# ceres-solver/ceres-solver

Hardware: NVIDIA H100
Metric: lm_iterations_per_sec (higher is better)
Workload: dtype f64

## Files before the change

ceres_solver_b200/csrc/explicit_schur.cuh:

```cuda
#pragma once
#include "common.cuh"

namespace b200 {

constexpr int kXsThreads = 256;
constexpr int kXsWarps = kXsThreads / 32;
constexpr int kXsMinCtas = 2;
constexpr int kXsStep = 3;
constexpr int kXsAsmThreads = 256;
constexpr int kXsLongPairs = 96;
constexpr int kXsStepCountShift = 27;
constexpr int kXsStepFirst = 1 << 29;
constexpr int kXsStepLast = 1 << 30;

struct XsView {
  int C;
  int num_blocks;
  const int* blk_row;
  const int* blk_col;
  const int* pair_ptr;
  const int2* pairs;
  const int2* cols;
  const int* col_ptr;
  const int2* steps;
// ... 65 lines not shown
                                                                   double* __restrict__ upper45) {
  __shared__ double s_part[kLong ? kXsAsmThreads / 32 : 1][81];
  const int lane = threadIdx.x & 31, warp = threadIdx.x >> 5;
  const bool owner = lane < 27;
  const int u = owner ? lane / 3 : 0, w0 = owner ? 3 * (lane - 3 * (lane / 3)) : 0;
  const int item0 = kLong ? static_cast<int>(blockIdx.x) : static_cast<int>(blockIdx.x) * (kXsAsmThreads / 32) + warp;
  const int items = kLong ? static_cast<int>(gridDim.x) : static_cast<int>(gridDim.x) * (kXsAsmThreads / 32);
  for (int it = item0; it < num; it += items) {
    const int b = __ldg(blocks + it);
    const int p0 = __ldg(v.pair_ptr + b), p1 = __ldg(v.pair_ptr + b + 1);
    double acc[3] = {0.0, 0.0, 0.0};
    if (kLong) {
      constexpr int W = kXsAsmThreads / 32;
      const int n = p1 - p0;
      xs_pairs(v, p, ete_inv, p0 + static_cast<int>(static_cast<long long>(n) * warp / W),
               p0 + static_cast<int>(static_cast<long long>(n) * (warp + 1) / W), lane, acc[0], acc[1], acc[2]);
      __syncthreads();
      if (owner)
#pragma unroll
        for (int m = 0; m < 3; ++m) s_part[warp][9 * u + w0 + m] = acc[m];
      __syncthreads();
      if (warp != 0) continue;
      if (owner)
#pragma unroll
        for (int m = 0; m < 3; ++m) {
          double t = 0.0;
#pragma unroll
          for (int k = 0; k < W; ++k) t += s_part[k][9 * u + w0 + m];
          acc[m] = t;
        }
    } else {
      xs_pairs(v, p, ete_inv, p0, p1, lane, acc[0], acc[1], acc[2]);
    }
    if (owner) {
      double* sb = v.S + 81 * static_cast<size_t>(b) + 9 * u + w0;
      sb[0] = acc[0];
      sb[1] = acc[1];
      sb[2] = acc[2];
      const int i = __ldg(v.blk_row + b);
      if (upper45 != nullptr && __ldg(v.blk_col + b) == i) {
        double* o = upper45 + 45 * static_cast<size_t>(i) + u * 9 - u * (u - 1) / 2 - u;
        if (u <= w0) o[w0] = acc[0];
        if (u <= w0 + 1) o[w0 + 1] = acc[1];
        if (u <= w0 + 2) o[w0 + 2] = acc[2];
      }
    }
  }
}

struct XsStepData {
  int2 d;
  int2 c;
  double s[9];
};
template <bool kShared>
__device__ __forceinline__ int2 xs_step_desc(const XsView& v, int k, int k1) {
  return k < k1 ? (kShared ? v.steps[k] : __ldg(v.steps + k)) : make_int2(0, 0);
}
__device__ __forceinline__ bool xs_lane_in(int2 d, int e) { return e < ((d.y >> kXsStepCountShift) & 3); }
template <bool kShared>
__device__ __forceinline__ int2 xs_step_col(const XsView& v, int2 d, int e) {
  return xs_lane_in(d, e) ? (kShared ? v.cols[d.x + e] : __ldg(v.cols + d.x + e)) : make_int2(0, -1);
}
__device__ __forceinline__ void xs_step_s(const XsView& v, int2 d, int e, int w, double* s) {
  const bool in = xs_lane_in(d, e);
  const int b = in ? d.x + e : 0;
  const double* sb = v.S + 81 * static_cast<size_t>(b) + w;
#pragma unroll
  for (int u = 0; u < 9; ++u) s[u] = in ? __ldg(sb + 9 * u) : 0.0;
}

struct XsWalk {
  XsStepData nx;
  int2 d2, c2;
};
template <bool kShared = false, class LoadS>
__device__ __forceinline__ void xs_walk_begin(const XsView& v, int k0, int k1, int e, int w, LoadS load_s, XsWalk& wk) {
  wk.nx.d = xs_step_desc<kShared>(v, k0, k1);
  wk.nx.c = xs_step_col<kShared>(v, wk.nx.d, e);
  load_s(wk.nx.d, e, w, wk.nx.s);
  wk.d2 = xs_step_desc<kShared>(v, k0 + 1, k1);
  wk.c2 = xs_step_col<kShared>(v, wk.d2, e);
}
template <bool kShared = false, class LoadS, class LoadX, class RowOut>
__device__ __forceinline__ double xs_walk(const XsView& v, int k0, int k1, int lane, int e, int w, LoadS load_s, LoadX load_x,
                                          RowOut row_out, XsWalk& wk) {
  XsStepData& nx = wk.nx;
  int2 d2 = wk.d2, c2 = wk.c2;
  double nx_x = xs_lane_in(nx.d, e) ? load_x(nx.c.x, w) : 0.0;
  double acc[9], xi[9];
#pragma unroll
  for (int u = 0; u < 9; ++u) acc[u] = xi[u] = 0.0;
  double pq = 0.0;
  for (int k = k0; k < k1; ++k) {
    const int2 d = nx.d, c = nx.c;
    double s[9];
#pragma unroll
    for (int u = 0; u < 9; ++u) s[u] = nx.s[u];
    const double xj = nx_x;
    nx.d = d2;
    nx.c = c2;
    load_s(nx.d, e, w, nx.s);
    nx_x = xs_lane_in(nx.d, e) ? load_x(nx.c.x, w) : 0.0;
    d2 = xs_step_desc<kShared>(v, k + 2, k1);
    c2 = xs_step_col<kShared>(v, d2, e);
    if (d.y & kXsStepFirst)
#pragma unroll
      for (int u = 0; u < 9; ++u) xi[u] = __shfl_sync(0xffffffffu, xj, u);
    double t = 0.0;
#pragma unroll
    for (int u = 0; u < 9; ++u) {
      acc[u] += s[u] * xj;
      t += s[u] * xi[u];
    }
    if (c.y >= 0) {
      v.T[9 * static_cast<size_t>(c.y) + w] = t;
      pq += xj * t;
    }
    if (d.y & kXsStepLast) {
      double mine = 0.0, xo = 0.0;
#pragma unroll
      for (int u = 0; u < 9; ++u) {
        double a = acc[u];
#pragma unroll
        for (int o = 16; o > 0; o >>= 1) a += __shfl_xor_sync(0xffffffffu, a, o);
        if (lane == u) {
          mine = a;
          xo = xi[u];
        }
        acc[u] = 0.0;
      }
      if (lane < 9) {
        pq += xo * mine;
        row_out(d.y & ((1 << kXsStepCountShift) - 1), lane, mine, xo);
      }
    }
  }
  return pq;
}

__global__ void __launch_bounds__(kXsThreads, kXsMinCtas) xs_mul_kernel(XsView v, const double* __restrict__ x, double* y,
                                                                        const double* __restrict__ Df, int accumulate,
                                                                        const int* __restrict__ done_flag, double* pq_part) {
  __shared__ double s_pq[kXsWarps];
  const int warp = threadIdx.x >> 5, lane = threadIdx.x & 31;
  const int e = lane / 9, w = lane - 9 * (lane / 9);
  const int gw = blockIdx.x * kXsWarps + warp;
  const int k0 = __ldg(v.warp_step + gw), k1 = __ldg(v.warp_step + gw + 1);
  auto load_s = [&](int2 d, int e, int w, double* s) { xs_step_s(v, d, e, w, s); };
  XsWalk wk;
  xs_walk_begin(v, k0, k1, e, w, load_s, wk);
  asm volatile("griddepcontrol.wait;" ::: "memory");
  if (done_flag != nullptr && __ldcg(done_flag) != 0) return;
  double pq = xs_walk(
      v, k0, k1, lane, e, w, load_s, [&](int j, int w) { return __ldcg(x + 9 * static_cast<size_t>(j) + w); },
      [&](int i, int u, double a, double xo) {
        const size_t o = 9 * static_cast<size_t>(i) + u;
        double out = a;
        if (Df != nullptr) out += Df[o] * Df[o] * xo;
        if (accumulate) out += __ldcg(y + o);
        y[o] = out;
      },
      wk);
  if (pq_part == nullptr) return;
#pragma unroll
  for (int o = 16; o > 0; o >>= 1) pq += __shfl_xor_sync(0xffffffffu, pq, o);
  if (lane == 0) s_pq[warp] = pq;
  __syncthreads();
  if (threadIdx.x == 0) {
    double tot = 0.0;
#pragma unroll
    for (int ww = 0; ww < kXsWarps; ++ww) tot += s_pq[ww];
    pq_part[blockIdx.x] = tot;
  }
}

template <bool kStaged>
__device__ __forceinline__ double xs_col_sum(const double* src, int base, int c0, int c1, int w, double q) {
  for (int c = c0; c < c1; c += 8) {
    double t[8];
#pragma unroll
    for (int m = 0; m < 8; ++m) {
      const double* s = src + 9 * static_cast<size_t>(c + m - base) + w;
      t[m] = c + m < c1 ? (kStaged ? *s : __ldcg(s)) : 0.0;
    }
#pragma unroll
    for (int m = 0; m < 8; ++m)
      if (c + m < c1) q += t[m];
  }
  return q;
}
__device__ __forceinline__ double xs_col_sum(const int* __restrict__ col_ptr, const double* T, int k, double q) {
  const int j = k / 9, w = k - 9 * (k / 9);
  return xs_col_sum<false>(T, 0, __ldg(col_ptr + j), __ldg(col_ptr + j + 1), w, q);
}

__global__ void __launch_bounds__(256) xs_gather_kernel(XsView v, double* y) {
  const int k = blockIdx.x * blockDim.x + threadIdx.x;
  if (k < 9 * v.C) y[k] = xs_col_sum(v.col_ptr, v.T, k, y[k]);
}

}
```

ceres_solver_b200/csrc/plan.cuh:

```cuda
#pragma once
#include <algorithm>
#include <cmath>
#include <cstdio>
#include <cstdlib>
#include <cstring>
#include <numeric>
#include <vector>

#include "explicit_schur.cuh"
#include "kernels_v4b.cuh"
#include "xs_pcg.cuh"

namespace b200 {

constexpr double kL2ResidentShare = 0.5;
constexpr double kXsByteRatio = 2.0;
constexpr double kXsMaxBytes = 128.0 * (1 << 20);

enum KernelId {
  K_EVAL_JAC = 0,
  K_EVAL_COST,
  K_SQNORM,
  K_SCALE,
  K_JMUL,
// ... 64 lines not shown
    if (const char* e = dev_env("B200_BIG_COST")) k.big_cost = std::max(0.0, atof(e));
    if (const char* e = dev_env("B200_DIRECT_LIMIT")) k.direct_limit = atol(e);
    if (const char* e = dev_env("B200_V3_WARPS")) k.v3_warps = atoi(e);
    if (const char* e = dev_env("B200_V3_REPLICAS")) k.v3_replicas = atoi(e);
    if (const char* e = dev_env("B200_V4_WARPS")) k.v4_warps = std::max(4, std::min(k.v4_warps, atoi(e)));
    if (const char* e = dev_env("B200_V4_STAGES")) k.v4_stages = std::max(1, std::min(3, atoi(e)));
    if (const char* e = dev_env("B200_V4_REPLICAS")) k.v4_replicas = std::max(1, atoi(e));
    if (const char* e = dev_env("B200_L2_RESIDENT_MB")) {
      k.l2_mb_set = true;
      k.l2_mb = atof(e);
    }
    if (const char* e = dev_env("B200_L2_RESIDENT_POLICY")) k.l2_last = strcmp(e, "last") == 0;
    if (const char* e = dev_env("B200_EXPLICIT_S")) k.explicit_s = atoi(e) != 0 ? 1 : 0;
    k.no_pdl = dev_env("B200_NO_PDL") != nullptr;
    k.no_fused_pq = dev_env("B200_NO_FUSED_PQ") != nullptr;
    k.no_peer_exchange = dev_env("B200_NO_PEER_EXCHANGE") != nullptr;
    if (const char* e = dev_env("B200_XS_RESIDENT")) k.xs_resident = atoi(e) != 0 ? 1 : 0;
    return k;
  }
};

struct DevLimits {
  int sm_count;
  size_t smem_optin;
  int l2_bytes;
  int xs_ctas_per_sm;
  int xs_pcg_ctas_per_sm;
};

enum class MulFamily { Tile, V3, V4, V4Owned };
enum class DiagPass { CamMajor, WarpTile, Tile };

inline bool is_v4(MulFamily m) { return m == MulFamily::V4 || m == MulFamily::V4Owned; }

struct XsPattern {
  long long off_blocks = 0;
  std::vector<int> blk_row, blk_col, pair_ptr, row_ptr, col_ptr;
  std::vector<int2> pairs, cols;
};

struct KernelPlan {
  int order_choice = 0;
  long order_metrics[4] = {0, 0, 0, 0};
  std::vector<int> pt_perm;
  std::vector<int> row_perm;
  std::vector<int> cam_idx, pt_idx, pt_ptr;
  std::vector<double> obs;
  std::vector<TileDesc> tiles;
  std::vector<TileDesc> chunk_tiles;
  std::vector<int> huge_pts;
  std::vector<WarpTile> wtiles;
  std::vector<TileDesc> big_tiles;
  int num_plain_big = 0;
  std::vector<uint32_t> row_meta;
  std::vector<int> cam_rows;
  std::vector<CamItem> cam_items;
  bool has_dups = false;
  int num_ctas = 0;
  std::vector<int2> cta_part, cta_cam, cta_big;
  std::vector<int> cta_cams;
  int max_cam_span = 1;
  MulFamily mul = MulFamily::Tile;
  DiagPass diag = DiagPass::Tile;
  bool big_folded = false;
  V2View v2{}, v2_mul{}, v2_eval{}, v2_diag{};
  size_t v2_smem = 0, mul_smem = 0, eval_smem = 0, diag_smem = 0;
  int diag_replicas = 0;
  std::vector<uint32_t> tile_meta;
  double l2_budget = 0.0, l2_stream_bytes = 0.0, l2_resident_bytes = 0.0;
  bool xs = false;
  XsPattern xp;
  std::vector<int> xs_order;
  std::vector<int2> xs_steps;
  std::vector<int> xs_warp_step;
  int num_xs_long = 0, xs_grid = 0, xs_resident = 0, xs_max_steps = 0;
  bool xs_pcg = false;
  std::vector<int2> xs_pcg_cta;
  std::vector<int> xs_pcg_warp_step;
  std::vector<int> xs_pcg_fptr;
  std::vector<int> xs_pcg_fcol;
  std::vector<int2> xs_pcg_cols;
  int xs_pcg_max_blocks = 0, xs_pcg_max_cams = 0, xs_pcg_max_steps = 0, xs_pcg_max_foreign = 0;
  int xs_pcg_max_cta_steps = 0;
  int xs_pcg_max_slots = 0;
  int xs_pcg_stage_slots = 0;
  size_t xs_pcg_smem = 0;
  const char* xs_pcg_why = "";
  double bytes_per_op[K_COUNT] = {};
};

inline void xs_pattern(int C, int N, const int* cam_idx, const int* pt_idx, const int* pt_ptr, XsPattern* xp) {
  std::vector<int> cptr(static_cast<size_t>(C) + 1, 0), crow(static_cast<size_t>(N));
  for (int r = 0; r < N; ++r) cptr[cam_idx[r] + 1]++;
  for (int c = 0; c < C; ++c) cptr[c + 1] += cptr[c];
  {
    std::vector<int> fill(cptr.begin(), cptr.end() - 1);
    for (int r = 0; r < N; ++r) crow[fill[cam_idx[r]]++] = r;
  }
  std::vector<int> stamp(static_cast<size_t>(C), -1), slot(static_cast<size_t>(C), 0), js, start;
  std::vector<int>& row_start = xp->row_ptr;
  row_start.assign(static_cast<size_t>(C) + 1, 0);
  std::vector<int3> tup;
  for (int i = 0; i < C; ++i) {
    js.clear();
    tup.clear();
    stamp[i] = i;
    js.push_back(i);
    for (int k = cptr[i]; k < cptr[i + 1]; ++k) {
      const int r = crow[k], p = pt_idx[r];
      for (int s = pt_ptr[p]; s < pt_ptr[p + 1]; ++s) {
        const int j = cam_idx[s];
        if (j < i) continue;
        if (stamp[j] != i) {
          stamp[j] = i;
          js.push_back(j);
        }
        tup.push_back(make_int3(j, r, s));
      }
    }
    std::sort(js.begin(), js.end());
    xp->off_blocks += static_cast<long long>(js.size()) - 1;
    row_start[i] = static_cast<int>(xp->blk_row.size());
    start.assign(js.size() + 1, 0);
    for (size_t t = 0; t < js.size(); ++t) {
      slot[js[t]] = static_cast<int>(t);
      xp->blk_row.push_back(i);
      xp->blk_col.push_back(js[t]);
    }
    for (const int3& t : tup) start[slot[t.x] + 1]++;
    for (size_t t = 0; t < js.size(); ++t) start[t + 1] += start[t];
    const size_t base = xp->pairs.size();
    for (size_t t = 0; t < js.size(); ++t) xp->pair_ptr.push_back(static_cast<int>(base + start[t]));
    xp->pairs.resize(base + tup.size());
    for (const int3& t : tup) xp->pairs[base + start[slot[t.x]]++] = make_int2(t.y, t.z);
  }
  const int nb = static_cast<int>(xp->blk_row.size());
  row_start[C] = nb;
  xp->pair_ptr.push_back(static_cast<int>(xp->pairs.size()));
  xp->col_ptr.assign(static_cast<size_t>(C) + 1, 0);
  for (int b = 0; b < nb; ++b)
    if (xp->blk_col[b] != xp->blk_row[b]) xp->col_ptr[xp->blk_col[b] + 1]++;
  for (int c = 0; c < C; ++c) xp->col_ptr[c + 1] += xp->col_ptr[c];
  std::vector<int> fill(xp->col_ptr.begin(), xp->col_ptr.end() - 1);
  xp->cols.resize(static_cast<size_t>(nb));
  for (int b = 0; b < nb; ++b)
    xp->cols[b] = make_int2(xp->blk_col[b], xp->blk_col[b] != xp->blk_row[b] ? fill[xp->blk_col[b]]++ : -1);
}

inline int xs_assembly_order(const XsPattern& xp, std::vector<int>* order) {
  const int nb = static_cast<int>(xp.blk_row.size());
  order->clear();
  order->reserve(static_cast<size_t>(nb));
  for (int b = 0; b < nb; ++b)
    if (xp.pair_ptr[b + 1] - xp.pair_ptr[b] > kXsLongPairs) order->push_back(b);
  const int num_long = static_cast<int>(order->size());
  for (int b = 0; b < nb; ++b)
    if (xp.pair_ptr[b + 1] - xp.pair_ptr[b] <= kXsLongPairs) order->push_back(b);
  return num_long;
}

const char* const kOrderNames[4] = {"caller's order kept", "by camera arc", "by mean camera", "by smallest camera"};
inline int choose_point_order(int C, int P, int N, const int32_t* cam_of_row, const int* caller_ptr, int chunks, std::vector<int>* perm,
                       long metrics[4]) {
  std::vector<int> ident(static_cast<size_t>(P));
  std::iota(ident.begin(), ident.end(), 0);
  auto metric = [&](const std::vector<int>& ord) -> long {
// ... 440 lines not shown
    if (knobs.explicit_s >= 0) pl.xs = knobs.explicit_s != 0 && npairs < 2.0e9;
    xs_asm_bytes = 196.0 * N + 48.0 * P + 8.0 * npairs + 12.0 * nb + 648.0 * nb + 360.0 * C;
  }
  if (pl.xs) {
    const XsPattern& xp = pl.xp;
    const int nb = static_cast<int>(xp.blk_row.size());
    pl.xs_resident = std::max(1, lim.xs_ctas_per_sm) * lim.sm_count;
    pl.xs_grid = std::max(1, std::min(pl.xs_resident, (C + kXsWarps - 1) / kXsWarps));
    const int nw = pl.xs_grid * kXsWarps;
    auto row_steps = [&](int i) { return (xp.row_ptr[i + 1] - xp.row_ptr[i] + kXsStep - 1) / kXsStep; };
    double total = 0.0;
    for (int i = 0; i < C; ++i) total += row_steps(i) + 1;
    pl.xs_warp_step.assign(static_cast<size_t>(nw) + 1, 0);
    double cum = 0.0;
    int w = 0;
    for (int i = 0; i < C; ++i) {
      const int owner = std::min(nw - 1, static_cast<int>(cum * nw / total));
      while (w < owner) pl.xs_warp_step[++w] = static_cast<int>(pl.xs_steps.size());
      const int r0 = xp.row_ptr[i], r1 = xp.row_ptr[i + 1];
      for (int b = r0; b < r1; b += kXsStep) {
        const int n = std::min(kXsStep, r1 - b);
        pl.xs_steps.push_back(make_int2(b, i | (n << kXsStepCountShift) | (b == r0 ? kXsStepFirst : 0) |
                                               (b + kXsStep >= r1 ? kXsStepLast : 0)));
      }
      cum += row_steps(i) + 1;
    }
    while (w < nw) pl.xs_warp_step[++w] = static_cast<int>(pl.xs_steps.size());
    for (int k = 0; k < nw; ++k) pl.xs_max_steps = std::max(pl.xs_max_steps, pl.xs_warp_step[k + 1] - pl.xs_warp_step[k]);
    {
      const int G = lim.sm_count;
      std::vector<int> first_step(static_cast<size_t>(C) + 1, 0);
      for (int i = 0; i < C; ++i) first_step[i + 1] = first_step[i] + row_steps(i);
      auto row_blocks = [&](int i) { return xp.row_ptr[i + 1] - xp.row_ptr[i]; };
      auto ctas_at = [&](int K) {
        int g = 1, cur = 0;
        for (int i = 0; i < C; ++i) {
          if (cur + row_blocks(i) > K) {
            ++g;
            cur = 0;
          }
          cur += row_blocks(i);
        }
        return g;
      };
      int lo = (nb + G - 1) / G, hi = nb;
      for (int i = 0; i < C; ++i) lo = std::max(lo, row_blocks(i));
      while (lo < hi) {
        const int mid = lo + (hi - lo) / 2;
        if (ctas_at(mid) <= G) hi = mid;
        else lo = mid + 1;
      }
      pl.xs_pcg_cta.assign(static_cast<size_t>(G) + 1, make_int2(C, nb));
      pl.xs_pcg_cta[0] = make_int2(0, 0);
      for (int i = 0, g = 0, cur = 0; i < C; ++i) {
        if (cur + row_blocks(i) > lo) {
          pl.xs_pcg_cta[++g] = make_int2(i, xp.row_ptr[i]);
          cur = 0;
        }
        cur += row_blocks(i);
      }
      pl.xs_pcg_warp_step.assign(static_cast<size_t>(G) * kXpWarps + 1, first_step[C]);
      pl.xs_pcg_fptr.assign(static_cast<size_t>(G) + 1, 0);
      pl.xs_pcg_cols.resize(static_cast<size_t>(nb));
      for (int b = 0; b < G; ++b) {
        const int i0 = pl.xs_pcg_cta[b].x, i1 = pl.xs_pcg_cta[b + 1].x;
        const int b0 = pl.xs_pcg_cta[b].y, b1 = pl.xs_pcg_cta[b + 1].y;
        pl.xs_pcg_max_blocks = std::max(pl.xs_pcg_max_blocks, b1 - b0);
        pl.xs_pcg_max_cams = std::max(pl.xs_pcg_max_cams, i1 - i0);
        pl.xs_pcg_max_cta_steps = std::max(pl.xs_pcg_max_cta_steps, first_step[i1] - first_step[i0]);
        pl.xs_pcg_max_slots = std::max(pl.xs_pcg_max_slots, xp.col_ptr[i1] - xp.col_ptr[i0]);
        std::vector<int> fc;
        for (int k = b0; k < b1; ++k)
          if (xp.blk_col[k] >= i1) fc.push_back(xp.blk_col[k]);
        std::sort(fc.begin(), fc.end());
        fc.erase(std::unique(fc.begin(), fc.end()), fc.end());
        for (int k = b0; k < b1; ++k) {
          const int j = xp.blk_col[k];
          const int l = j < i1 ? j - i0 : (i1 - i0) + static_cast<int>(std::lower_bound(fc.begin(), fc.end(), j) - fc.begin());
          pl.xs_pcg_cols[k] = make_int2(l, xp.cols[k].y);
        }
        pl.xs_pcg_fcol.insert(pl.xs_pcg_fcol.end(), fc.begin(), fc.end());
        pl.xs_pcg_fptr[b + 1] = static_cast<int>(pl.xs_pcg_fcol.size());
        pl.xs_pcg_max_foreign = std::max(pl.xs_pcg_max_foreign, static_cast<int>(fc.size()));
        double tot = 0.0, cum = 0.0;
        for (int i = i0; i < i1; ++i) tot += row_steps(i) + 1;
        int* ws = pl.xs_pcg_warp_step.data() + static_cast<size_t>(b) * kXpWarps;
        int wv = 0;
        ws[0] = first_step[i0];
        for (int i = i0; i < i1; ++i) {
          const int owner = std::min(kXpWarps - 1, static_cast<int>(cum * kXpWarps / tot));
          while (wv < owner) ws[++wv] = first_step[i];
          cum += row_steps(i) + 1;
        }
        while (wv < kXpWarps - 1) ws[++wv] = first_step[i1];
      }
      for (int k = 0; k < G * kXpWarps; ++k)
        pl.xs_pcg_max_steps = std::max(pl.xs_pcg_max_steps, pl.xs_pcg_warp_step[k + 1] - pl.xs_pcg_warp_step[k]);
      const size_t base = xs_pcg_smem_bytes(pl.xs_pcg_max_blocks, pl.xs_pcg_max_cams, pl.xs_pcg_max_foreign, pl.xs_pcg_max_cta_steps, 0);
      const size_t room = lim.smem_optin > base + 1024 ? lim.smem_optin - base - 1024 : 0;
      pl.xs_pcg_stage_slots = static_cast<int>(std::min<size_t>(pl.xs_pcg_max_slots, room / (9 * sizeof(double))));
      pl.xs_pcg_smem = xs_pcg_smem_bytes(pl.xs_pcg_max_blocks, pl.xs_pcg_max_cams, pl.xs_pcg_max_foreign, pl.xs_pcg_max_cta_steps,
                                         pl.xs_pcg_stage_slots);
      if (pl.xs_pcg_smem + 1024 > lim.smem_optin) pl.xs_pcg_why = "largest CTA's shared memory exceeds the limit";
      else if (lim.xs_pcg_ctas_per_sm < 1) pl.xs_pcg_why = "no CTA of the kernel fits an SM";
      else if (knobs.xs_resident == 0) pl.xs_pcg_why = "B200_XS_RESIDENT=0";
      else pl.xs_pcg = true;
    }
    pl.num_xs_long = xs_assembly_order(xp, &pl.xs_order);
  }

  const double Nn = N, Pp = P, Cc = C;
  double* bpo = pl.bytes_per_op;
  bpo[K_JTJ] = 196 * Nn + 4 * Pp + 24.0 * (3 * Pp + 9 * Cc);
  bpo[K_SCHUR_MUL] = 196 * Nn + 52 * Pp + 216 * Cc;
  bpo[K_SCHUR_INIT] = 196 * Nn + 16 * Nn + 4 * Pp + 24 * Pp + 48 * Pp + 72 * Cc;
  bpo[K_DIAG_BLOCKS] = 196 * Nn + 52 * Pp + 360 * Cc;
  bpo[K_BACKSUB] = 196 * Nn + 16 * Nn + 52 * Pp + 24 * Pp + 72 * Cc;
  bpo[K_EVAL_JAC] = 192 * Nn + 16 * Nn + 16 * Nn + 4 * Nn + 4 * Pp + 2 * 8.0 * (3 * Pp + 9 * Cc);
  bpo[K_EVAL_COST] = 16 * Nn + 4 * Nn + 4 * Pp + 8.0 * (3 * Pp + 9 * Cc);
  bpo[K_SQNORM] = 196 * Nn + 4 * Pp + 8.0 * (3 * Pp + 9 * Cc);
  bpo[K_SCALE] = 2 * 192 * Nn + 8 * Nn + 8.0 * (3 * Pp + 9 * Cc);
  bpo[K_JMUL] = 196 * Nn + 32 * Nn + 4 * Pp + 8.0 * (3 * Pp + 9 * Cc);
  bpo[K_JTMUL] = 196 * Nn + 16 * Nn + 4 * Pp + 16.0 * (3 * Pp + 9 * Cc);
  bpo[K_PMV_RIGHT_E] = 48 * Nn + 4 * Nn + 32 * Nn + 24 * Pp;
  bpo[K_PMV_RIGHT_F] = 144 * Nn + 4 * Nn + 32 * Nn + 72 * Cc;
  bpo[K_PMV_LEFT_E] = 48 * Nn + 16 * Nn + 4 * Pp + 48 * Pp;
  bpo[K_PMV_LEFT_F] = 144 * Nn + 16 * Nn + 4 * Nn + 144 * Cc;
  bpo[K_MODEL_COST] = 196 * Nn + 16 * Nn + 4 * Pp + 8.0 * (3 * Pp + 9 * Cc);
  bpo[K_DOGLEG_GRAM] = 196 * Nn + 4 * Pp + 16.0 * (3 * Pp + 9 * Cc);
  bpo[K_DOGLEG_DIAG] = 48.0 * (3 * Pp + 9 * Cc);
  bpo[K_DOGLEG_GN] = 32.0 * (3 * Pp + 9 * Cc);
  bpo[K_DOGLEG_STEP] = 56.0 * (3 * Pp + 9 * Cc);
  if (pl.xs) {
    bpo[K_SCHUR_MUL] = xs_mul_bytes;
    bpo[K_DIAG_BLOCKS] = xs_asm_bytes;
    const double nb = static_cast<double>(pl.xp.blk_row.size()), off = static_cast<double>(pl.xp.off_blocks);
    if (pl.xs_pcg) bpo[K_SCHUR_PCG] = 656.0 * nb + 144.0 * off + 648.0 * Cc + 8 * 72.0 * Cc;
  }
}

inline void print_plan(const KernelPlan& pl, int C, int P, int N, int world, const DevLimits& lim, const DevKnobs& knobs) {
  if (getenv("B200_VERBOSE") == nullptr) return;
  if (!knobs.keep_order)
    fprintf(stderr, "[b200ba] point order: distinct cameras per 1/%d of the rows, summed: caller %ld, by camera arc %ld, by mean camera %ld, by smallest camera %ld -> %s\n",
            lim.sm_count, pl.order_metrics[0], pl.order_metrics[1], pl.order_metrics[2], pl.order_metrics[3], kOrderNames[pl.order_choice]);
  const V2View &v = pl.v2, &m = pl.v2_mul;
  if (is_v4(pl.mul)) {
    const uint32_t s = m.l2_stream;
    fprintf(stderr, "[b200ba] S*x L2 plan (L2 %d MiB, budget %.1f MiB): resident %.1f MiB, streamed %.1f MiB, stride %.2f tiles (%s)\n",
            lim.l2_bytes >> 20, pl.l2_budget / (1 << 20), pl.l2_resident_bytes / (1 << 20), (pl.l2_stream_bytes - pl.l2_resident_bytes) / (1 << 20),
            s < 65536 ? 65536.0 / (65536 - s) : 0.0, m.l2_last ? "evict_last" : "evict_normal");
  }
  const char* const mul_names[] = {"tile", "v3", "v4", "v4-owned"};
  const char* const diag_names[] = {"cam_major", "v2", "tile"};
  fprintf(stderr,
          "[b200ba] C=%d P=%d N=%d wtiles=%zu big(+slices)=%zu huge=%d span=%d direct=%d v2(w=%d,s=%d,r=%d) mul(%s w=%d,s=%d,r=%d,smem=%zu) folded=%d v2b=%d cam_major=%d diag=%s\n",
          C, P, N, pl.wtiles.size(), pl.big_tiles.size(), static_cast<int>(pl.huge_pts.size()), pl.max_cam_span, v.direct, v.warps, v.stages,
          v.replicas, mul_names[static_cast<int>(pl.mul)], m.warps, m.stages, m.replicas, pl.mul_smem, pl.big_folded ? 1 : 0,
          is_v4(pl.mul) ? 1 : 0, pl.diag == DiagPass::CamMajor ? 1 : 0, diag_names[static_cast<int>(pl.diag)]);
  if (world == 1) {
    fprintf(stderr, "[b200ba] S plan: %s, %lld pairs, %.1f MB\n", pl.xs ? "explicit" : "implicit", pl.xp.off_blocks,
            648.0 * static_cast<double>(pl.xp.blk_row.size()) / 1e6);
    if (pl.xs)
      fprintf(stderr, "[b200ba] S product: grid %d of %d resident CTAs (%d per SM), %d warps, at most %d steps per warp\n",
              pl.xs_grid, pl.xs_resident, lim.xs_ctas_per_sm, pl.xs_grid * kXsWarps, pl.xs_max_steps);
    if (pl.xs) {
      const double share = 648.0 * pl.xs_pcg_max_blocks / 1024.0, limit = static_cast<double>(lim.smem_optin) / 1024.0;
      const double cta = static_cast<double>(pl.xs_pcg_smem) / 1024.0;
      if (pl.xs_pcg)
        fprintf(stderr, "[b200ba] S PCG: resident, %d CTAs, largest S share %.2f KiB of %.2f KiB (%.2f KiB with M^-1, vectors and staging), %d warps, at most %d steps per warp, at most %d foreign columns, at most %d column slots per CTA (%d staged)\n",
                lim.sm_count, share, limit, cta, lim.sm_count * kXpWarps, pl.xs_pcg_max_steps, pl.xs_pcg_max_foreign, pl.xs_pcg_max_slots,
                pl.xs_pcg_stage_slots);
      else
        fprintf(stderr, "[b200ba] S PCG: two-kernel (%s: largest S share %.2f KiB, %.2f KiB with M^-1, vectors and staging, of %.2f KiB)\n",
                pl.xs_pcg_why, share, cta, limit);
    }
  } else
    fprintf(stderr, "[b200ba] S plan: implicit, sharded\n");
}

}
```

ceres_solver_b200/csrc/xs_pcg.cuh:

```cuda
#pragma once
#include "cg_kernel.cuh"

namespace b200 {

constexpr int kXpThreads = 512;
constexpr int kXpWarps = kXpThreads / 32;
inline size_t xs_pcg_smem_bytes(int max_blocks, int max_cams, int max_foreign, int max_steps, int slots) {
  return sizeof(double) * (81 * static_cast<size_t>(max_blocks) + (81 + 7 * 9) * static_cast<size_t>(max_cams) +
                           9 * static_cast<size_t>(max_cams + max_foreign) + 9 * static_cast<size_t>(slots)) +
         sizeof(int2) * (static_cast<size_t>(max_steps) + static_cast<size_t>(max_blocks)) +
         sizeof(int) * (static_cast<size_t>(max_cams) + 1 + static_cast<size_t>(max_foreign));
}

struct XsPcgArgs {
  XsView v;
  CgParams prm;
  int reset;
  const int2* cta;
  const int* warp_step;
  const int* fptr;
  const int* fcol;
  int max_blocks, max_cams;
  int max_foreign;
  int max_steps;
  int stage_slots;
  const double* minv;
  const double* rhs;
  const double* Df;
  double *x, *z;
  double* p[2];
  double* red;
  CgState* st;
#ifdef B200_DEV_KNOBS
  long long* stamps;
#endif
};

constexpr int kXpPhases = 6;
#ifdef B200_DEV_KNOBS
#define XP_STAMP(k)                                                   \
  if (a.stamps != nullptr && blockIdx.x == 0 && threadIdx.x == 0) {   \
    const long long t_now = clock64();                                \
    a.stamps[k] += t_now - t_mark;                                    \
    t_mark = t_now;                                                   \
  }
#else
#define XP_STAMP(k)
#endif

__global__ void __launch_bounds__(kXpThreads, 1) xs_pcg_kernel(XsPcgArgs a) {
  cg::grid_group grid = cg::this_grid();
#ifdef B200_DEV_KNOBS
  long long t_mark = clock64();
#endif
  extern __shared__ double smem[];
  __shared__ double scratch[kXpWarps][3];
  __shared__ double s_tot[4];
  __shared__ int s_nfe;
  const int tid = threadIdx.x, warp = tid >> 5, lane = tid & 31;
  const int e = lane / 9, w = lane - 9 * (lane / 9);
  const int2 lo = a.cta[blockIdx.x], hi = a.cta[blockIdx.x + 1];
  const int r0 = lo.x, ncam = hi.x - lo.x, nent = 9 * ncam, b0 = lo.y, nblk = hi.y - lo.y;
  double* s_S = smem;
  double* s_minv = s_S + 81 * static_cast<size_t>(a.max_blocks);
  double* s_x = s_minv + 81 * static_cast<size_t>(a.max_cams);
  double* s_r = s_x + 9 * a.max_cams;
  double* s_p = s_r + 9 * a.max_cams;
  double* s_b = s_p + 9 * a.max_cams;
  double* s_d = s_b + 9 * a.max_cams;
  double* s_a = s_d + 9 * a.max_cams;
  double* s_z = s_a + 9 * a.max_cams;
  double* s_v = s_z + 9 * a.max_cams;
  double* s_T = s_v + 9 * (a.max_cams + a.max_foreign);
  int2* s_steps = reinterpret_cast<int2*>(s_T + 9 * a.stage_slots);
  int2* s_cols = s_steps + a.max_steps;
  int* s_cp = reinterpret_cast<int*>(s_cols + a.max_blocks);
  int* s_fc = s_cp + a.max_cams + 1;
  const XsView& v = a.v;
  const int kc = __ldg(a.warp_step + blockIdx.x * kXpWarps);
  XsView vs = v;
  vs.steps = s_steps - kc;
  vs.cols = s_cols - b0;
  const size_t o0 = 9 * static_cast<size_t>(r0);
  const bool writer = blockIdx.x == 0 && tid == 0;
  const int k0 = __ldg(a.warp_step + blockIdx.x * kXpWarps + warp), k1 = __ldg(a.warp_step + blockIdx.x * kXpWarps + warp + 1);

  {
    const double* src = v.S + 81 * static_cast<size_t>(b0);
    const int n = 81 * nblk;
    int i = tid;
    for (; i + 3 * kXpThreads < n; i += 4 * kXpThreads) {
      double t[4];
#pragma unroll
      for (int k = 0; k < 4; ++k) t[k] = __ldcg(src + i + k * kXpThreads);
#pragma unroll
      for (int k = 0; k < 4; ++k) s_S[i + k * kXpThreads] = t[k];
    }
    for (; i < n; i += kXpThreads) s_S[i] = __ldcg(src + i);
    for (int k = tid; k < 81 * ncam; k += kXpThreads) s_minv[k] = __ldcg(a.minv + 81 * static_cast<size_t>(r0) + k);
    for (int k = tid; k <= ncam; k += kXpThreads) s_cp[k] = __ldg(v.col_ptr + r0 + k);
    const int nsteps = __ldg(a.warp_step + (blockIdx.x + 1) * kXpWarps) - kc;
    for (int k = tid; k < nsteps; k += kXpThreads) s_steps[k] = __ldg(v.steps + kc + k);
    for (int k = tid; k < nblk; k += kXpThreads) s_cols[k] = __ldg(v.cols + b0 + k);
    const int f0 = __ldg(a.fptr + blockIdx.x), nf = __ldg(a.fptr + blockIdx.x + 1) - f0;
    for (int k = tid; k < nf; k += kXpThreads) s_fc[k] = __ldg(a.fcol + f0 + k);
    if (tid == 0) s_nfe = 9 * nf;
  }
  for (int k = tid; k < nent; k += kXpThreads) {
    s_b[k] = a.rhs[o0 + k];
    s_d[k] = a.Df != nullptr ? a.Df[o0 + k] : 0.0;
    s_p[k] = 0.0;
  }
  auto load_s = [&](int2 d, int e, int w, double* s) {
    const bool in = xs_lane_in(d, e);
    const double* sb = s_S + 81 * (in ? d.x + e - b0 : 0) + w;
#pragma unroll
    for (int u = 0; u < 9; ++u) s[u] = in ? sb[9 * u] : 0.0;
  };
  auto keep_row = [&](int i, int u, double av, double) { s_a[9 * (i - r0) + u] = av; };
  auto staged = [&]() { return s_cp[ncam] - s_cp[0] <= a.stage_slots; };
  auto stage_T = [&]() {
    if (!staged()) return;
    const int c0 = s_cp[0];
    const double* src = v.T + 9 * static_cast<size_t>(c0);
    const int n = 9 * (s_cp[ncam] - c0);
    int i = tid;
    for (; i + 7 * kXpThreads < n; i += 8 * kXpThreads) {
      double t[8];
#pragma unroll
      for (int k = 0; k < 8; ++k) t[k] = __ldcg(src + i + k * kXpThreads);
#pragma unroll
      for (int k = 0; k < 8; ++k) s_T[i + k * kXpThreads] = t[k];
    }
    for (; i < n; i += kXpThreads) s_T[i] = __ldcg(src + i);
  };
  auto col_sum = [&](bool from_s, int k, double init) {
    const int cl = k / 9;
    return from_s ? xs_col_sum<true>(s_T, s_cp[0], s_cp[cl], s_cp[cl + 1], k - 9 * cl, init)
                  : xs_col_sum(v.col_ptr, v.T, static_cast<int>(o0) + k, init);
  };
  auto precondition = [&]() {
    __syncthreads();
    double accQ = 0.0, accR = 0.0, accRho = 0.0;
    for (int k = tid; k < nent; k += kXpThreads) {
      const int cl = k / 9, row = k - 9 * cl;
      const double* m = s_minv + 81 * cl + 9 * row;
      const double* rc = s_r + 9 * cl;
      double zj = 0.0;
#pragma unroll
      for (int t = 0; t < 9; ++t) zj += m[t] * rc[t];
      s_z[k] = zj;
      a.z[o0 + k] = zj;
      const double xj = s_x[k], rj = s_r[k];
      accQ += xj * (s_b[k] + rj);
      accR += rj * rj;
      accRho += rj * zj;
    }
    cg_block_sum3<kXpWarps>(accQ, accR, accRho, scratch);
    if (tid == 0) {
      a.red[blockIdx.x * 4 + 1] = accQ;
      a.red[blockIdx.x * 4 + 2] = accR;
      a.red[blockIdx.x * 4 + 3] = accRho;
    }
  };

  for (int k = tid; k < nent; k += kXpThreads) {
    s_x[k] = 0.0;
    s_r[k] = s_b[k];
    a.x[o0 + k] = 0.0;
  }
  precondition();
  grid.sync();
  double tot[3];
  cg_totals(a.red, gridDim.x, 1, 3, tot, s_tot);
  XP_STAMP(0);
  double rho = 1.0, Q0 = 0.0, tol_r = 0.0, beta = 0.0;
  int it = 0;
  if (!cg_phase_c(a.prm, true, 0, rho, Q0, tol_r, tot[0], tot[1], tot[2], a.st, writer, &beta, &Q0, &tol_r)) return;
  rho = tot[2];

  for (;;) {
    double pq = 0.0;
    const double* p_prev = a.p[it & 1];
    for (int k = tid; k < nent + s_nfe; k += kXpThreads) {
      if (k < nent) {
        const double pn = cg_next_p(it, s_z[k], beta, s_p[k]);
        s_p[k] = pn;
        s_v[k] = pn;
        a.p[(it + 1) & 1][o0 + k] = pn;
        pq += s_d[k] * s_d[k] * pn * pn;
      } else {
        const int fl = (k - nent) / 9;
        const size_t o = 9 * static_cast<size_t>(s_fc[fl]) + (k - nent - 9 * fl);
        s_v[k] = cg_next_p(it, __ldcg(a.z + o), beta, __ldcg(p_prev + o));
      }
    }
    ++it;
    __syncthreads();
    {
      XsWalk wk;
      xs_walk_begin<true>(vs, k0, k1, e, w, load_s, wk);
      pq += xs_walk<true>(vs, k0, k1, lane, e, w, load_s, [&](int l, int w) { return s_v[9 * l + w]; }, keep_row, wk);
    }
    {
      double d1 = 0.0, d2 = 0.0;
      cg_block_sum3<kXpWarps>(pq, d1, d2, scratch);
      if (tid == 0) a.red[blockIdx.x * 4] = pq;
    }
    XP_STAMP(1);
    grid.sync();
    XP_STAMP(2);
    double pq_tot, alpha = 0.0;
    const bool reset = it % a.reset == 0;
    if (!reset) stage_T();
    cg_totals(a.red, gridDim.x, 0, 1, &pq_tot, s_tot);
    if (!cg_alpha(pq_tot, rho, it, a.st, writer, &alpha)) return;
    const bool from_s = staged();
    for (int k = tid; k < nent; k += kXpThreads) {
      const double pj = s_p[k];
      double xj = s_x[k];
      xj += alpha * pj;
      s_x[k] = xj;
      a.x[o0 + k] = xj;
      if (reset) {
        s_v[k] = xj;
      } else {
        const double dj = s_d[k];
        const double q = col_sum(from_s, k, __dadd_rn(s_a[k], __dmul_rn(__dmul_rn(dj, dj), pj)));
        double rj = s_r[k];
        rj -= alpha * q;
        s_r[k] = rj;
      }
    }
    if (reset) {
      grid.sync();
      for (int k = tid; k < s_nfe; k += kXpThreads) {
        const int fl = k / 9;
        s_v[nent + k] = __ldcg(a.x + 9 * static_cast<size_t>(s_fc[fl]) + (k - 9 * fl));
      }
      __syncthreads();
      {
        XsWalk wk;
        xs_walk_begin<true>(vs, k0, k1, e, w, load_s, wk);
        xs_walk<true>(vs, k0, k1, lane, e, w, load_s, [&](int l, int w) { return s_v[9 * l + w]; }, keep_row, wk);
      }
      grid.sync();
      stage_T();
      __syncthreads();
      for (int k = tid; k < nent; k += kXpThreads) {
        const double dj = s_d[k];
        const double q = col_sum(from_s, k, __dadd_rn(s_a[k], __dmul_rn(__dmul_rn(dj, dj), s_x[k])));
        s_r[k] = s_b[k] - q;
      }
    }
    precondition();
    XP_STAMP(3);
    grid.sync();
    XP_STAMP(4);
    cg_totals(a.red, gridDim.x, 1, 3, tot, s_tot);
    if (!cg_phase_c(a.prm, false, it, rho, Q0, tol_r, tot[0], tot[1], tot[2], a.st, writer, &beta, &Q0, &tol_r)) return;
    rho = tot[2];
    XP_STAMP(5);
  }
}

}
```

Baseline: 142.7.

## Split Schur rows across warps with segment joins, transpose smem S, prefetch foreign p

The persistent PCG kernel now gives each warp a balanced share of steps, found by binary search on a per-step cost. A row may be split across warps, so partial row sums go to a per-warp segment buffer and are joined after the walk. It also stores the S blocks transposed in shared memory so the per-lane loads are contiguous, and prefetches the foreign z/p values into registers right after the grid sync. This aims to cut warp load imbalance and shared-memory bank conflicts, at the cost of extra join logic, shared memory and synchronisation.

```diff
diff --git a/ceres_solver_b200/csrc/explicit_schur.cuh b/ceres_solver_b200/csrc/explicit_schur.cuh
--- a/ceres_solver_b200/csrc/explicit_schur.cuh
+++ b/ceres_solver_b200/csrc/explicit_schur.cuh
@@ -171,15 +171,19 @@
   wk.d2 = xs_step_desc<kShared>(v, k0 + 1, k1);
   wk.c2 = xs_step_col<kShared>(v, wk.d2, e);
 }
-template <bool kShared = false, class LoadS, class LoadX, class RowOut>
+constexpr int kXsStepRowMask = (1 << kXsStepCountShift) - 1;
+template <bool kShared = false, class LoadS, class LoadX, class LoadXi, class RowOut>
 __device__ __forceinline__ double xs_walk(const XsView& v, int k0, int k1, int lane, int e, int w, LoadS load_s, LoadX load_x,
-                                          RowOut row_out, XsWalk& wk) {
+                                          LoadXi load_xi, RowOut row_out, XsWalk& wk) {
   XsStepData& nx = wk.nx;
   int2 d2 = wk.d2, c2 = wk.c2;
   double nx_x = xs_lane_in(nx.d, e) ? load_x(nx.c.x, w) : 0.0;
   double acc[9], xi[9];
 #pragma unroll
   for (int u = 0; u < 9; ++u) acc[u] = xi[u] = 0.0;
+  if (k0 < k1 && !(nx.d.y & kXsStepFirst))
+#pragma unroll
+    for (int u = 0; u < 9; ++u) xi[u] = load_xi(nx.d.y & kXsStepRowMask, u);
   double pq = 0.0;
   for (int k = k0; k < k1; ++k) {
     const int2 d = nx.d, c = nx.c;
@@ -206,7 +210,7 @@
       v.T[9 * static_cast<size_t>(c.y) + w] = t;
       pq += xj * t;
     }
-    if (d.y & kXsStepLast) {
+    if ((d.y & kXsStepLast) || k + 1 == k1) {
       double mine = 0.0, xo = 0.0;
 #pragma unroll
       for (int u = 0; u < 9; ++u) {
@@ -221,7 +225,7 @@
       }
       if (lane < 9) {
         pq += xo * mine;
-        row_out(d.y & ((1 << kXsStepCountShift) - 1), lane, mine, xo);
+        row_out(d.y & kXsStepRowMask, lane, mine, xo);
       }
     }
   }
@@ -241,8 +245,9 @@
   xs_walk_begin(v, k0, k1, e, w, load_s, wk);
   asm volatile("griddepcontrol.wait;" ::: "memory");
   if (done_flag != nullptr && __ldcg(done_flag) != 0) return;
+  auto load_x = [&](int j, int w) { return __ldcg(x + 9 * static_cast<size_t>(j) + w); };
   double pq = xs_walk(
-      v, k0, k1, lane, e, w, load_s, [&](int j, int w) { return __ldcg(x + 9 * static_cast<size_t>(j) + w); },
+      v, k0, k1, lane, e, w, load_s, load_x, load_x,
       [&](int i, int u, double a, double xo) {
         const size_t o = 9 * static_cast<size_t>(i) + u;
         double out = a;
diff --git a/ceres_solver_b200/csrc/plan.cuh b/ceres_solver_b200/csrc/plan.cuh
--- a/ceres_solver_b200/csrc/plan.cuh
+++ b/ceres_solver_b200/csrc/plan.cuh
@@ -170,6 +170,8 @@
   std::vector<int2> xs_pcg_cols;
   int xs_pcg_max_blocks = 0, xs_pcg_max_cams = 0, xs_pcg_max_steps = 0, xs_pcg_max_foreign = 0;
   int xs_pcg_max_cta_steps = 0;
+  int xs_pcg_walk_max = 0;
+  int xs_pcg_split_rows = 0;
   int xs_pcg_max_slots = 0;
   int xs_pcg_stage_slots = 0;
   size_t xs_pcg_smem = 0;
@@ -776,17 +778,40 @@
         pl.xs_pcg_fcol.insert(pl.xs_pcg_fcol.end(), fc.begin(), fc.end());
         pl.xs_pcg_fptr[b + 1] = static_cast<int>(pl.xs_pcg_fcol.size());
         pl.xs_pcg_max_foreign = std::max(pl.xs_pcg_max_foreign, static_cast<int>(fc.size()));
-        double tot = 0.0, cum = 0.0;
-        for (int i = i0; i < i1; ++i) tot += row_steps(i) + 1;
+        const int s0 = first_step[i0], s1 = first_step[i1];
+        auto fill = [&](int K, int* ws) {
+          int g = 0, cost = 0;
+          if (ws != nullptr) ws[0] = s0;
+          for (int k = s0; k < s1; ++k) {
+            const bool row_start = (pl.xs_steps[k].y & kXsStepFirst) != 0;
+            if (cost + 1 + (row_start || cost == 0) > K) {
+              if (++g == kXpWarps) return g + 1;
+              if (ws != nullptr) ws[g] = k;
+              cost = 0;
+            }
+            cost += 1 + (row_start || cost == 0);
+          }
+          if (ws != nullptr)
+            while (g < kXpWarps - 1) ws[++g] = s1;
+          return g + 1;
+        };
+        int klo = 2, khi = std::max(2, 2 * (s1 - s0));
+        while (klo < khi) {
+          const int mid = klo + (khi - klo) / 2;
+          if (fill(mid, nullptr) <= kXpWarps) khi = mid;
+          else klo = mid + 1;
+        }
         int* ws = pl.xs_pcg_warp_step.data() + static_cast<size_t>(b) * kXpWarps;
-        int wv = 0;
-        ws[0] = first_step[i0];
-        for (int i = i0; i < i1; ++i) {
-          const int owner = std::min(kXpWarps - 1, static_cast<int>(cum * kXpWarps / tot));
-          while (wv < owner) ws[++wv] = first_step[i];
-          cum += row_steps(i) + 1;
-        }
-        while (wv < kXpWarps - 1) ws[++wv] = first_step[i1];
+        fill(klo, ws);
+        for (int wv = 0; wv < kXpWarps; ++wv) {
+          const int ka = ws[wv], kb = wv + 1 < kXpWarps ? ws[wv + 1] : s1;
+          if (ka == kb) continue;
+          int cost = kb - ka + 1;
+          for (int k = ka + 1; k < kb; ++k) cost += (pl.xs_steps[k].y & kXsStepFirst) != 0;
+          pl.xs_pcg_walk_max = std::max(pl.xs_pcg_walk_max, cost);
+          const int df = pl.xs_steps[ka].y, dl = pl.xs_steps[kb - 1].y;
+          if (!(dl & kXsStepLast) && ((df & kXsStepFirst) || (df & kXsStepRowMask) != (dl & kXsStepRowMask))) ++pl.xs_pcg_split_rows;
+        }
       }
       for (int k = 0; k < G * kXpWarps; ++k)
         pl.xs_pcg_max_steps = std::max(pl.xs_pcg_max_steps, pl.xs_pcg_warp_step[k + 1] - pl.xs_pcg_warp_step[k]);
@@ -861,13 +886,16 @@
     if (pl.xs) {
       const double share = 648.0 * pl.xs_pcg_max_blocks / 1024.0, limit = static_cast<double>(lim.smem_optin) / 1024.0;
       const double cta = static_cast<double>(pl.xs_pcg_smem) / 1024.0;
-      if (pl.xs_pcg)
+      if (pl.xs_pcg) {
         fprintf(stderr, "[b200ba] S PCG: resident, %d CTAs, largest S share %.2f KiB of %.2f KiB (%.2f KiB with M^-1, vectors and staging), %d warps, at most %d steps per warp, at most %d foreign columns, at most %d column slots per CTA (%d staged)\n",
                 lim.sm_count, share, limit, cta, lim.sm_count * kXpWarps, pl.xs_pcg_max_steps, pl.xs_pcg_max_foreign, pl.xs_pcg_max_slots,
                 pl.xs_pcg_stage_slots);
-      else
+        fprintf(stderr, "[b200ba] S PCG walk: at most %d steps per warp (one per row segment included), %d split rows\n",
+                pl.xs_pcg_walk_max, pl.xs_pcg_split_rows);
+      } else {
         fprintf(stderr, "[b200ba] S PCG: two-kernel (%s: largest S share %.2f KiB, %.2f KiB with M^-1, vectors and staging, of %.2f KiB)\n",
                 pl.xs_pcg_why, share, cta, limit);
+      }
     }
   } else
     fprintf(stderr, "[b200ba] S plan: implicit, sharded\n");
diff --git a/ceres_solver_b200/csrc/xs_pcg.cuh b/ceres_solver_b200/csrc/xs_pcg.cuh
--- a/ceres_solver_b200/csrc/xs_pcg.cuh
+++ b/ceres_solver_b200/csrc/xs_pcg.cuh
@@ -7,9 +7,9 @@
 constexpr int kXpWarps = kXpThreads / 32;
 inline size_t xs_pcg_smem_bytes(int max_blocks, int max_cams, int max_foreign, int max_steps, int slots) {
   return sizeof(double) * (81 * static_cast<size_t>(max_blocks) + (81 + 7 * 9) * static_cast<size_t>(max_cams) +
-                           9 * static_cast<size_t>(max_cams + max_foreign) + 9 * static_cast<size_t>(slots)) +
+                           9 * static_cast<size_t>(max_cams + max_foreign) + 9 * kXpWarps + 9 * static_cast<size_t>(slots)) +
          sizeof(int2) * (static_cast<size_t>(max_steps) + static_cast<size_t>(max_blocks)) +
-         sizeof(int) * (static_cast<size_t>(max_cams) + 1 + static_cast<size_t>(max_foreign));
+         sizeof(int) * (static_cast<size_t>(max_cams) + 1 + static_cast<size_t>(max_foreign) + kXpWarps + 1);
 }
 
 struct XsPcgArgs {
@@ -71,11 +71,13 @@
   double* s_a = s_d + 9 * a.max_cams;
   double* s_z = s_a + 9 * a.max_cams;
   double* s_v = s_z + 9 * a.max_cams;
-  double* s_T = s_v + 9 * (a.max_cams + a.max_foreign);
+  double* s_seg = s_v + 9 * (a.max_cams + a.max_foreign);
+  double* s_T = s_seg + 9 * kXpWarps;
   int2* s_steps = reinterpret_cast<int2*>(s_T + 9 * a.stage_slots);
   int2* s_cols = s_steps + a.max_steps;
   int* s_cp = reinterpret_cast<int*>(s_cols + a.max_blocks);
   int* s_fc = s_cp + a.max_cams + 1;
+  int* s_ws = s_fc + a.max_foreign;
   const XsView& v = a.v;
   const int kc = __ldg(a.warp_step + blockIdx.x * kXpWarps);
   XsView vs = v;
@@ -88,15 +90,19 @@
   {
     const double* src = v.S + 81 * static_cast<size_t>(b0);
     const int n = 81 * nblk;
+    auto transposed = [](int i) {
+      const int b = i / 81, uw = i - 81 * b, u = uw / 9;
+      return 81 * b + 9 * (uw - 9 * u) + u;
+    };
     int i = tid;
     for (; i + 3 * kXpThreads < n; i += 4 * kXpThreads) {
       double t[4];
 #pragma unroll
       for (int k = 0; k < 4; ++k) t[k] = __ldcg(src + i + k * kXpThreads);
 #pragma unroll
-      for (int k = 0; k < 4; ++k) s_S[i + k * kXpThreads] = t[k];
-    }
-    for (; i < n; i += kXpThreads) s_S[i] = __ldcg(src + i);
+      for (int k = 0; k < 4; ++k) s_S[transposed(i + k * kXpThreads)] = t[k];
+    }
+    for (; i < n; i += kXpThreads) s_S[transposed(i)] = __ldcg(src + i);
     for (int k = tid; k < 81 * ncam; k += kXpThreads) s_minv[k] = __ldcg(a.minv + 81 * static_cast<size_t>(r0) + k);
     for (int k = tid; k <= ncam; k += kXpThreads) s_cp[k] = __ldg(v.col_ptr + r0 + k);
     const int nsteps = __ldg(a.warp_step + (blockIdx.x + 1) * kXpWarps) - kc;
@@ -105,6 +111,7 @@
     const int f0 = __ldg(a.fptr + blockIdx.x), nf = __ldg(a.fptr + blockIdx.x + 1) - f0;
     for (int k = tid; k < nf; k += kXpThreads) s_fc[k] = __ldg(a.fcol + f0 + k);
     if (tid == 0) s_nfe = 9 * nf;
+    if (tid <= kXpWarps) s_ws[tid] = __ldg(a.warp_step + blockIdx.x * kXpWarps + tid);
   }
   for (int k = tid; k < nent; k += kXpThreads) {
     s_b[k] = a.rhs[o0 + k];
@@ -113,11 +120,35 @@
   }
   auto load_s = [&](int2 d, int e, int w, double* s) {
     const bool in = xs_lane_in(d, e);
-    const double* sb = s_S + 81 * (in ? d.x + e - b0 : 0) + w;
-#pragma unroll
-    for (int u = 0; u < 9; ++u) s[u] = in ? sb[9 * u] : 0.0;
-  };
-  auto keep_row = [&](int i, int u, double av, double) { s_a[9 * (i - r0) + u] = av; };
+    const double* sb = s_S + 81 * (xs_lane_in(d, 0) ? d.x + (in ? e : 0) - b0 : 0) + 9 * w;
+#pragma unroll
+    for (int u = 0; u < 9; ++u) s[u] = in ? sb[u] : 0.0;
+  };
+  auto load_xi = [&](int i, int u) { return s_v[9 * (i - r0) + u]; };
+  auto keep_row = [&](int i, int u, double av, double) {
+    const int2 d0 = vs.steps[k0];
+    if (!(d0.y & kXsStepFirst) && (d0.y & kXsStepRowMask) == i) s_seg[9 * warp + u] = av;
+    else s_a[9 * (i - r0) + u] = av;
+  };
+  auto join_rows = [&]() {
+    if (tid >= 9 * kXpWarps) return;
+    const int wv = tid / 9, u = tid - 9 * wv;
+    const int ka = s_ws[wv], kb = s_ws[wv + 1];
+    if (ka == kb) return;
+    const int2 dl = vs.steps[kb - 1], df = vs.steps[ka];
+    const int i = dl.y & kXsStepRowMask;
+    if ((dl.y & kXsStepLast) || (!(df.y & kXsStepFirst) && (df.y & kXsStepRowMask) == i)) return;
+    double* out = s_a + 9 * (i - r0) + u;
+    double acc = *out;
+    for (int w2 = wv + 1; w2 < kXpWarps; ++w2) {
+      const int kb2 = s_ws[w2 + 1];
+      if (s_ws[w2] == kb2) continue;
+      acc += s_seg[9 * w2 + u];
+      const int2 d2 = vs.steps[kb2 - 1];
+      if ((d2.y & kXsStepLast) || (d2.y & kXsStepRowMask) != i) break;
+    }
+    *out = acc;
+  };
   auto staged = [&]() { return s_cp[ncam] - s_cp[0] <= a.stage_slots; };
   auto stage_T = [&]() {
     if (!staged()) return;
@@ -169,13 +200,23 @@
     s_r[k] = s_b[k];
     a.x[o0 + k] = 0.0;
   }
+  int it = 0;
+  double fz = 0.0, fp = 0.0;
+  auto prefetch_foreign = [&]() {
+    const int k = tid - nent;
+    if (k < 0 || k >= s_nfe) return;
+    const int fl = k / 9;
+    const size_t o = 9 * static_cast<size_t>(s_fc[fl]) + (k - 9 * fl);
+    fz = __ldcg(a.z + o);
+    fp = __ldcg(a.p[it & 1] + o);
+  };
   precondition();
   grid.sync();
+  prefetch_foreign();
   double tot[3];
   cg_totals(a.red, gridDim.x, 1, 3, tot, s_tot);
   XP_STAMP(0);
   double rho = 1.0, Q0 = 0.0, tol_r = 0.0, beta = 0.0;
-  int it = 0;
   if (!cg_phase_c(a.prm, true, 0, rho, Q0, tol_r, tot[0], tot[1], tot[2], a.st, writer, &beta, &Q0, &tol_r)) return;
   rho = tot[2];
 
@@ -189,6 +230,8 @@
         s_v[k] = pn;
         a.p[(it + 1) & 1][o0 + k] = pn;
         pq += s_d[k] * s_d[k] * pn * pn;
+      } else if (k < kXpThreads) {
+        s_v[k] = cg_next_p(it, fz, beta, fp);
       } else {
         const int fl = (k - nent) / 9;
         const size_t o = 9 * static_cast<size_t>(s_fc[fl]) + (k - nent - 9 * fl);
@@ -200,13 +243,14 @@
     {
       XsWalk wk;
       xs_walk_begin<true>(vs, k0, k1, e, w, load_s, wk);
-      pq += xs_walk<true>(vs, k0, k1, lane, e, w, load_s, [&](int l, int w) { return s_v[9 * l + w]; }, keep_row, wk);
+      pq += xs_walk<true>(vs, k0, k1, lane, e, w, load_s, [&](int l, int w) { return s_v[9 * l + w]; }, load_xi, keep_row, wk);
     }
     {
       double d1 = 0.0, d2 = 0.0;
       cg_block_sum3<kXpWarps>(pq, d1, d2, scratch);
       if (tid == 0) a.red[blockIdx.x * 4] = pq;
     }
+    join_rows();
     XP_STAMP(1);
     grid.sync();
     XP_STAMP(2);
@@ -242,8 +286,10 @@
       {
         XsWalk wk;
         xs_walk_begin<true>(vs, k0, k1, e, w, load_s, wk);
-        xs_walk<true>(vs, k0, k1, lane, e, w, load_s, [&](int l, int w) { return s_v[9 * l + w]; }, keep_row, wk);
-      }
+        xs_walk<true>(vs, k0, k1, lane, e, w, load_s, [&](int l, int w) { return s_v[9 * l + w]; }, load_xi, keep_row, wk);
+      }
+      __syncthreads();
+      join_rows();
       grid.sync();
       stage_T();
       __syncthreads();
@@ -256,6 +302,7 @@
     precondition();
     XP_STAMP(3);
     grid.sync();
+    prefetch_foreign();
     XP_STAMP(4);
     cg_totals(a.red, gridDim.x, 1, 3, tot, s_tot);
     if (!cg_phase_c(a.prm, false, it, rho, Q0, tol_r, tot[0], tot[1], tot[2], a.st, writer, &beta, &Q0, &tol_r)) return;
```

New measurement: 150.6, median of 6. +5.5%, better.
